# YuemingJin/STswinCL

Hardware: AMD Instinct MI355X
Metric: input frames/s, TswinPlus fwd+bwd+Adam, 4-frame 512x512 clips (higher is better)
Workload: dtype bf16; 1 GPU; BASELINE.json configs[1]: TswinPlus(12) seg train step, 4 clips/GPU x T=4 frames x 3x512x512, swin res (64,64), OHEM-CE, Adam; T=4 because the reference asserts it (swin_512.py:313); clips_per_gpu=4, frames_per_clip=4, parallelism=dp1, graph_requested=True

## Files before the change

### stswincl_amd/csrc/headops.hip

```cpp
#include "common.h"
#include <cstdlib>

static int reduce_rows_per_chunk(int group_rows, int other_blocks, int nrl) {
  int rpc = 8 * nrl;
  while (rpc < 64 * nrl && (long)other_blocks * ((group_rows + 2 * rpc - 1) / (2 * rpc)) >= 1024) rpc *= 2;
  return rpc;
}
static int bn_bwd_rows(long rows_all_groups, int col_blocks, int nrl, int max_rows) {
  static const int tgt_red = getenv("STSWIN_BN_RED_WGS") ? atoi(getenv("STSWIN_BN_RED_WGS")) : 512;
  static const int tgt_dx = getenv("STSWIN_BN_DX_WGS") ? atoi(getenv("STSWIN_BN_DX_WGS")) : 2048;
  const int tgt = max_rows > 32 ? tgt_red : tgt_dx;
  int rows = 8;
  while (rows < max_rows && (long)col_blocks * (rows_all_groups / ((long)2 * rows * nrl)) >= tgt) rows *= 2;
  return rows;
}

DEVI long group_row0(int g, int ch, int rows_per_chunk, int group_rows, int unit, int G) {
  if (unit <= 0) return (long)g * group_rows;
  return ((long)((ch * rows_per_chunk) / unit) * (G - 1) + g) * unit;
}
DEVI long group_first_row(int g, int group_rows, int unit) { return unit > 0 ? (long)g * unit : (long)g * group_rows; }
static int fit_chunk(int rpc, int unit) {
  if (unit <= 0) return rpc;
  while (rpc > 1 && unit % rpc) rpc >>= 1;
// ... 301 lines not shown
  w1 = s - (float)i0;
}

template <typename T>
__global__ __launch_bounds__(256) void bilinear_fwd_kernel(const T* in, long ldi, T* out, long ldo, int F, int h, int w,
                                                            int H, int W, int C) {
  constexpr int PACK = TT<T>::PACK;
  const int ppr = C / PACK;
  const long idx = (long)blockIdx.x * 256 + threadIdx.x;
  if (idx >= (long)F * H * W * ppr) return;
  const int c = (idx % ppr) * PACK;
  const long px = idx / ppr;
  const int x = px % W, y = (px / W) % H, f = px / ((long)W * H);
  int y0, y1, x0, x1; float wy, wx;
  bil_src(y, (float)h / H, h, y0, y1, wy);
  bil_src(x, (float)w / W, w, x0, x1, wx);
  const T* b = in + ((long)f * h * w) * ldi + c;
  Vec16<T> p00, p01, p10, p11, o;
  p00.v = *(const decltype(o.v)*)(b + ((long)y0 * w + x0) * ldi);
  p01.v = *(const decltype(o.v)*)(b + ((long)y0 * w + x1) * ldi);
  p10.v = *(const decltype(o.v)*)(b + ((long)y1 * w + x0) * ldi);
  p11.v = *(const decltype(o.v)*)(b + ((long)y1 * w + x1) * ldi);
#pragma unroll
  for (int e = 0; e < PACK; ++e)
    o.set(e, (1.f - wy) * ((1.f - wx) * p00.get(e) + wx * p01.get(e)) + wy * ((1.f - wx) * p10.get(e) + wx * p11.get(e)));
  *(decltype(o.v)*)(out + px * ldo + c) = o.v;
}

template <typename T>
__global__ __launch_bounds__(256) void bilinear_bwd_kernel(const T* dout, long ldo, T* din, long ldi, int F, int h, int w,
                                                            int H, int W, int C) {
  constexpr int PACK = TT<T>::PACK;
  const int ppr = C / PACK;
  const long idx = (long)blockIdx.x * 256 + threadIdx.x;
  if (idx >= (long)F * h * w * ppr) return;
  const int c = (idx % ppr) * PACK;
  const long px = idx / ppr;
  const int xi = px % w, yi = (px / w) % h, f = px / ((long)w * h);
  const float sy = (float)h / H, sx = (float)w / W;
  const int ylo = max(0, (int)floorf(((float)yi - 0.5f) / sy - 0.5f) - 1), yhi = min(H - 1, (int)ceilf(((float)yi + 1.5f) / sy - 0.5f) + 1);
  const int xlo = max(0, (int)floorf(((float)xi - 0.5f) / sx - 0.5f) - 1), xhi = min(W - 1, (int)ceilf(((float)xi + 1.5f) / sx - 0.5f) + 1);
  float acc[8] = {0, 0, 0, 0, 0, 0, 0, 0};
  for (int y = ylo; y <= yhi; ++y) {
    int y0, y1; float wy;
    bil_src(y, sy, h, y0, y1, wy);
    const float cy = (y0 == yi ? 1.f - wy : 0.f) + (y1 == yi ? wy : 0.f);
    if (cy == 0.f) continue;
    for (int x = xlo; x <= xhi; ++x) {
      int x0, x1; float wx;
      bil_src(x, sx, w, x0, x1, wx);
      const float cx = (x0 == xi ? 1.f - wx : 0.f) + (x1 == xi ? wx : 0.f);
      if (cx == 0.f) continue;
      Vec16<T> d;
      d.v = *(const decltype(d.v)*)(dout + (((long)f * H + y) * W + x) * ldo + c);
#pragma unroll
      for (int e = 0; e < PACK; ++e) acc[e] += cy * cx * d.get(e);
    }
  }
  Vec16<T> o;
#pragma unroll
  for (int e = 0; e < PACK; ++e) o.set(e, acc[e]);
  *(decltype(o.v)*)(din + px * ldi + c) = o.v;
}

template <typename T, typename TO>
__global__ __launch_bounds__(256) void logits_up_fwd_kernel(const T* in, long ldi, TO* out, int F, int h, int w, int H, int W,
                                                             int nc) {
  const long px = (long)blockIdx.x * 256 + threadIdx.x;
  if (px >= (long)F * H * W) return;
  const int x = px % W, y = (px / W) % H, f = px / ((long)W * H);
  int y0, y1, x0, x1; float wy, wx;
  bil_src(y, (float)h / H, h, y0, y1, wy);
  bil_src(x, (float)w / W, w, x0, x1, wx);
  const T* b = in + ((long)f * h * w) * ldi;
  const T* p00 = b + ((long)y0 * w + x0) * ldi; const T* p01 = b + ((long)y0 * w + x1) * ldi;
  const T* p10 = b + ((long)y1 * w + x0) * ldi; const T* p11 = b + ((long)y1 * w + x1) * ldi;
  for (int c = 0; c < nc; ++c) {
    const float v = (1.f - wy) * ((1.f - wx) * to_f32<T>(p00[c]) + wx * to_f32<T>(p01[c])) +
                    wy * ((1.f - wx) * to_f32<T>(p10[c]) + wx * to_f32<T>(p11[c]));
    out[(((long)f * nc + c) * H + y) * W + x] = from_f32<TO>(v);
  }
}

template <typename T, typename TO>
__global__ __launch_bounds__(256) void logits_up_bwd_kernel(const TO* dout, T* din, long ldi, int F, int h, int w, int H, int W,
                                                             int nc) {
  const long idx = (long)blockIdx.x * 256 + threadIdx.x;
  const long npx = (long)F * h * w;
  if (idx >= npx * nc) return;
  const int c = (int)(idx / npx);
  const long px = idx - (long)c * npx;
  const int xi = px % w, yi = (px / w) % h, f = px / ((long)w * h);
  const float sy = (float)h / H, sx = (float)w / W;
  const int ylo = max(0, (int)floorf(((float)yi - 0.5f) / sy - 0.5f) - 1), yhi = min(H - 1, (int)ceilf(((float)yi + 1.5f) / sy - 0.5f) + 1);
  const int xlo = max(0, (int)floorf(((float)xi - 0.5f) / sx - 0.5f) - 1), xhi = min(W - 1, (int)ceilf(((float)xi + 1.5f) / sx - 0.5f) + 1);
  const TO* plane = dout + ((long)f * nc + c) * H * W;
  float acc = 0.f;
  for (int y = ylo; y <= yhi; ++y) {
    int y0, y1; float wy;
    bil_src(y, sy, h, y0, y1, wy);
    const float cy = (y0 == yi ? 1.f - wy : 0.f) + (y1 == yi ? wy : 0.f);
    if (cy == 0.f) continue;
    float row = 0.f;
    for (int x = xlo; x <= xhi; ++x) {
      int x0, x1; float wx;
      bil_src(x, sx, w, x0, x1, wx);
      const float cx = (x0 == xi ? 1.f - wx : 0.f) + (x1 == xi ? wx : 0.f);
      if (cx != 0.f) row += cx * to_f32<TO>(plane[(long)y * W + x]);
    }
    acc += cy * row;
  }
  din[px * ldi + c] = from_f32<T>(acc);
}

DEVI unsigned long long loss_to_fix(float v) { return (unsigned long long)((double)fmaxf(v, 0.f) * 4294967296.0); }
DEVI float fix_to_loss(unsigned long long f) { return (float)((double)f * (1.0 / 4294967296.0)); }

template <typename TL>
__global__ __launch_bounds__(256) void ce_fwd_kernel(const TL* logits, const long* labels, float* loss, float* stats, int F,
                                                      long HW, int nc, int ignore_index, float thresh) {
  float hc = 0.f, hs = 0.f, nbad = 0.f;
  const long n = (long)F * HW;
  for (long px = (long)blockIdx.x * 256 + threadIdx.x; px < n; px += (long)gridDim.x * 256) {
    float l = 0.f;
    const long f = px / HW, p = px % HW;
    const long lab = labels[px];
    if (lab != ignore_index && (lab < 0 || lab >= nc)) {
      l = __builtin_nanf("");
      nbad += 1.f;
    } else if (lab != ignore_index) {
      const TL* b = logits + f * nc * HW + p;
      float mx = -3.0e38f;
      int am = 0;
      for (int c = 0; c < nc; ++c) {
        const float v = to_f32<TL>(b[(long)c * HW]);
        if (v > mx) { mx = v; am = c; }
      }
      float s = 0.f;
      for (int c = 0; c < nc; ++c)
        if (c != am) s += expf(to_f32<TL>(b[(long)c * HW]) - mx);
      l = (mx - to_f32<TL>(b[lab * HW])) + log1pf(s);
    }
    loss[px] = l;
    if (l > thresh) { hc += 1.f; hs += l; }
  }
  float cnt = wave_sum(hc), sm = wave_sum(hs), bad = wave_sum(nbad);
  __shared__ float red[3][4];
  if ((threadIdx.x & 63) == 0) { red[0][threadIdx.x >> 6] = cnt; red[1][threadIdx.x >> 6] = sm; red[2][threadIdx.x >> 6] = bad; }
  __syncthreads();
  if (threadIdx.x == 0) {
    const float nb = red[2][0] + red[2][1] + red[2][2] + red[2][3];
    if (nb != 0.f) atomicAdd(stats + 1, nb);
    atomicAdd(stats + 0, red[0][0] + red[0][1] + red[0][2] + red[0][3]);
    atomicAdd((unsigned long long*)(stats + 2), loss_to_fix(red[1][0] + red[1][1] + red[1][2] + red[1][3]));
  }
}

template <typename TL>
__global__ __launch_bounds__(256) void ce_bwd_kernel(const TL* logits, const long* labels, const float* loss, const float* sel,
                                                      const float* gscale, TL* dlogits, int F, long HW, int nc,
                                                      int ignore_index) {
  const long px = (long)blockIdx.x * 256 + threadIdx.x;
  if (px >= (long)F * HW) return;
  const long f = px / HW, p = px % HW;
  const long lab = labels[px];
  const float l = loss[px];
  const float w = l > sel[0] ? sel[1] : (l == sel[0] ? sel[3] : 0.f);
  const float wgt = (w != 0.f && lab != ignore_index && lab >= 0 && lab < nc) ? w * gscale[0] : 0.f;
  const TL* b = logits + f * nc * HW + p;
  TL* d = dlogits + f * nc * HW + p;
  if (wgt == 0.f) {
    for (int c = 0; c < nc; ++c) d[(long)c * HW] = from_f32<TL>(0.f);
    return;
  }
  float mx = -3.0e38f;
  for (int c = 0; c < nc; ++c) mx = fmaxf(mx, to_f32<TL>(b[(long)c * HW]));
  float s = 0.f;
  for (int c = 0; c < nc; ++c) s += expf(to_f32<TL>(b[(long)c * HW]) - mx);
  const float inv = 1.f / s;
  for (int c = 0; c < nc; ++c) {
    const float pr = expf(to_f32<TL>(b[(long)c * HW]) - mx) * inv;
    d[(long)c * HW] = from_f32<TL>(wgt * (pr - (c == lab ? 1.f : 0.f)));
  }
}

#define PACK_OF(dt) ((dt) == 0 ? 8 : 4)
#define DISPATCH_T(dt, CALL_BF16, CALL_F32) do { if ((dt) == 0) { CALL_BF16; } else { CALL_F32; } } while (0)

static int colstats_geometry(int dtype, int M, int C, int groups, int unit_rows, int* cpb_o, int* rpc_o, int* cpg_o) {
  if (C % PACK_OF(dtype) || groups <= 0 || M % groups) return -1401;
  if (unit_rows > 0 && M % ((long)groups * unit_rows)) return -1405;
  const int ppr = C / PACK_OF(dtype), cpb = pick_cpb(ppr);
  const int gr = M / groups, rpc = fit_chunk(reduce_rows_per_chunk(gr, groups * ((ppr + cpb - 1) / cpb), 256 / cpb), unit_rows);
  if (rpc <= 0) return -1405;
  *cpb_o = cpb; *rpc_o = rpc; *cpg_o = (gr + rpc - 1) / rpc;
  return 0;
}
extern "C" long stswin_colstats_scratch(int dtype, int M, int C, int groups, int unit_rows) {
  int cpb, rpc, cpg;
  const int rc = colstats_geometry(dtype, M, C, groups, unit_rows, &cpb, &rpc, &cpg);
  return rc ? rc : (long)groups * cpg * 2 * C;
}

extern "C" int stswin_colstats(int dtype, const void* x, long ldx, float* sum, float* sumsq, int M, int C, int groups,
                               int unit_rows, float* scratch, void* stream) {
  int cpb, rpc, cpg;
  const int rc = colstats_geometry(dtype, M, C, groups, unit_rows, &cpb, &rpc, &cpg);
  if (rc) return rc;
  if (ldx % PACK_OF(dtype)) return -1401;
  if (!scratch) return -1406;
  const int ppr = C / PACK_OF(dtype), gr = M / groups;
  dim3 grid((ppr + cpb - 1) / cpb, groups * cpg);
  hipStream_t st = (hipStream_t)stream;
  if (sumsq)
    DISPATCH_T(dtype, hipLaunchKernelGGL((colstats_kernel<bf16, true>), grid, dim3(256), 0, st, (const bf16*)x, ldx, scratch, C, gr, cpg, rpc, cpb, unit_rows),
               hipLaunchKernelGGL((colstats_kernel<float, true>), grid, dim3(256), 0, st, (const float*)x, ldx, scratch, C, gr, cpg, rpc, cpb, unit_rows));
  else
    DISPATCH_T(dtype, hipLaunchKernelGGL((colstats_kernel<bf16, false>), grid, dim3(256), 0, st, (const bf16*)x, ldx, scratch, C, gr, cpg, rpc, cpb, unit_rows),
               hipLaunchKernelGGL((colstats_kernel<float, false>), grid, dim3(256), 0, st, (const float*)x, ldx, scratch, C, gr, cpg, rpc, cpb, unit_rows));
  const int rf = stswin_fold_launch(scratch, 2L * C, (long)cpg * 2 * C, cpg, C, sumsq ? 2 : 1, sum, sumsq, nullptr, C, groups, 1, st);
  if (rf) return rf;
  STSWIN_CHECK_LAUNCH();
  return 0;
}

extern "C" int stswin_bn_finalize(int dtype, const void* x, long ldx, const float* sum, const float* sumsq, float* mean,
                                  float* rstd, float* running_mean, float* running_var, int M, int C, int groups, float eps,
                                  float momentum, int unit_rows, void* stream) {
  if (groups <= 0 || M % groups) return -1401;
  hipStream_t st = (hipStream_t)stream;
  dim3 grid((C + 255) / 256);
  DISPATCH_T(dtype, hipLaunchKernelGGL(bn_finalize_kernel<bf16>, grid, dim3(256), 0, st, (const bf16*)x, ldx, sum, sumsq, mean, rstd, running_mean, running_var, C, groups, M / groups, eps, momentum, unit_rows),
             hipLaunchKernelGGL(bn_finalize_kernel<float>, grid, dim3(256), 0, st, (const float*)x, ldx, sum, sumsq, mean, rstd, running_mean, running_var, C, groups, M / groups, eps, momentum, unit_rows));
  STSWIN_CHECK_LAUNCH();
  return 0;
}

extern "C" int stswin_bn_apply(int dtype, const void* x, long ldx, const float* mean, const float* rstd, const float* gamma,
                               const float* beta, const void* resid, long ldr, void* y, long ldy, int M, int C, int groups,
                               int relu, int unit_rows, void* stream) {
  const int pk = PACK_OF(dtype);
  if (C % pk || ldx % pk || ldy % pk || (resid && ldr % pk) || groups <= 0 || M % groups) return -1402;
  const int ppr = C / pk, cpb = pick_cpb(ppr);
  if (unit_rows > 0 && M % ((long)groups * unit_rows)) return -1405;
  const int gr = M / groups, rpc = fit_chunk(8 * (256 / cpb), unit_rows);
  if (rpc <= 0) return -1405;
  const int cpg = (gr + rpc - 1) / rpc;
  dim3 grid((ppr + cpb - 1) / cpb, groups * cpg);
  hipStream_t st = (hipStream_t)stream;
  DISPATCH_T(dtype, hipLaunchKernelGGL(bn_apply_kernel<bf16>, grid, dim3(256), 0, st, (const bf16*)x, ldx, mean, rstd, gamma, beta, (const bf16*)resid, ldr, (bf16*)y, ldy, C, gr, cpg, rpc, relu, cpb, unit_rows),
             hipLaunchKernelGGL(bn_apply_kernel<float>, grid, dim3(256), 0, st, (const float*)x, ldx, mean, rstd, gamma, beta, (const float*)resid, ldr, (float*)y, ldy, C, gr, cpg, rpc, relu, cpb, unit_rows));
  STSWIN_CHECK_LAUNCH();
  return 0;
}

static int bn_bwd_geometry(int dtype, int M, int C, int groups, int unit_rows, int* cpb_o, int* rpc_o, int* rpc2_o) {
  const int pk = PACK_OF(dtype);
  if (C % pk || groups <= 0 || M % groups) return -1403;
  if (unit_rows > 0 && M % ((long)groups * unit_rows)) return -1405;
  const int ppr = C / pk, cpb = pick_cpb(ppr), xb = (ppr + cpb - 1) / cpb, nrl = 256 / cpb;
  const int rpc = fit_chunk(bn_bwd_rows(M, xb, nrl, 64) * nrl, unit_rows);
  const int rpc2 = fit_chunk(bn_bwd_rows(M, xb, nrl, 32) * nrl, unit_rows);
  if (rpc <= 0 || rpc2 <= 0) return -1405;
  *cpb_o = cpb; *rpc_o = rpc; *rpc2_o = rpc2;
  return 0;
}
extern "C" long stswin_bn_bwd_scratch(int dtype, int M, int C, int groups, int unit_rows) {
  int cpb, rpc, rpc2;
  const int rc = bn_bwd_geometry(dtype, M, C, groups, unit_rows, &cpb, &rpc, &rpc2);
// ... 77 lines not shown
          const int kx = ix - 2 * ox;
          if (kx < 0 || kx > 2) continue;
          const int o = oy * 2 + ox;
          const unsigned char t = (unsigned char)(ky * 3 + kx);
#pragma unroll
          for (int e = 0; e < PACK; ++e) {
            const float u = z.get(e);
            if (u > best[o][e] || ba[o][e] == 255) { best[o][e] = u; ba[o][e] = t; }
          }
        }
      }
    }
  }
#pragma unroll
  for (int oy = 0; oy < 2; ++oy)
#pragma unroll
    for (int ox = 0; ox < 2; ++ox) {
      const int yo = 2 * yb + oy, xo = 2 * xb + ox, o = oy * 2 + ox;
      if (yo >= Hp || xo >= Wp) continue;
      const long px = (f * Hp + yo) * Wp + xo;
      Vec16<T> r;
      unsigned a[2] = {0, 0};
#pragma unroll
      for (int e = 0; e < PACK; ++e) { r.set(e, best[o][e]); a[e >> 2] |= (unsigned)ba[o][e] << (8 * (e & 3)); }
      if (PACK == 8) *(uint2*)(arg + px * C + c) = uint2{a[0], a[1]};
      else *(unsigned*)(arg + px * C + c) = a[0];
      *(decltype(r.v)*)(out + px * ldo + c) = r.v;
    }
}

extern "C" int stswin_bn_relu_pool(int dtype, const void* x, long ldx, const float* mean, const float* rstd, const float* gamma,
                                   const float* beta, void* out, long ldo, unsigned char* arg, int frames, int H, int W, int C, int groups,
                                   int unit_rows, void* stream) {
  const int pk = PACK_OF(dtype);
  const long M = (long)frames * H * W;
  if (frames <= 0 || H <= 0 || W <= 0 || C % pk || ldx % pk || ldo % pk || groups <= 0 || M % groups) return -1408;
  if (unit_rows > 0 ? (unit_rows % ((long)H * W) != 0 || M % ((long)groups * unit_rows)) : ((M / groups) % ((long)H * W) != 0)) return -1408;
  const int Hp = (H - 1) / 2 + 1, Wp = (W - 1) / 2 + 1;
  const long n = (long)frames * ((Hp + 1) / 2) * ((Wp + 1) / 2) * (C / pk);
  dim3 grid((unsigned)((n + 255) / 256));
  hipStream_t st = (hipStream_t)stream;
  DISPATCH_T(dtype, hipLaunchKernelGGL(bn_relu_pool_kernel<bf16>, grid, dim3(256), 0, st, (const bf16*)x, ldx, mean, rstd, gamma, beta, (bf16*)out, ldo, arg, frames, H, W, Hp, Wp, C, groups, (int)(M / groups), unit_rows),
             hipLaunchKernelGGL(bn_relu_pool_kernel<float>, grid, dim3(256), 0, st, (const float*)x, ldx, mean, rstd, gamma, beta, (float*)out, ldo, arg, frames, H, W, Hp, Wp, C, groups, (int)(M / groups), unit_rows));
  STSWIN_CHECK_LAUNCH();
  return 0;
}

extern "C" int stswin_rows_broadcast(int dtype, const float* v, void* out, long ldo, int M, int C, int groups, float scale,
                                     int accumulate, void* stream) {
  const int pk = PACK_OF(dtype);
  if (C % pk || ldo % pk || groups <= 0 || M % groups) return -1404;
  const long n = (long)M * (C / pk);
  dim3 grid((unsigned)((n + 255) / 256));
  hipStream_t st = (hipStream_t)stream;
  DISPATCH_T(dtype, hipLaunchKernelGGL(rows_broadcast_kernel<bf16>, grid, dim3(256), 0, st, v, (bf16*)out, ldo, M, C, M / groups, scale, accumulate),
             hipLaunchKernelGGL(rows_broadcast_kernel<float>, grid, dim3(256), 0, st, v, (float*)out, ldo, M, C, M / groups, scale, accumulate));
  STSWIN_CHECK_LAUNCH();
  return 0;
}

extern "C" int stswin_bilinear(int dtype, const void* in, long ldi, void* out, long ldo, int frames, int h, int w, int H, int W,
                               int C, int backward, void* stream) {
  const int pk = PACK_OF(dtype);
  if (C % pk || ldi % pk || ldo % pk) return -1405;
  hipStream_t st = (hipStream_t)stream;
  if (!backward) {
    const long n = (long)frames * H * W * (C / pk);
    dim3 grid((unsigned)((n + 255) / 256));
    DISPATCH_T(dtype, hipLaunchKernelGGL(bilinear_fwd_kernel<bf16>, grid, dim3(256), 0, st, (const bf16*)in, ldi, (bf16*)out, ldo, frames, h, w, H, W, C),
               hipLaunchKernelGGL(bilinear_fwd_kernel<float>, grid, dim3(256), 0, st, (const float*)in, ldi, (float*)out, ldo, frames, h, w, H, W, C));
  } else {
    const long n = (long)frames * h * w * (C / pk);
    dim3 grid((unsigned)((n + 255) / 256));
    DISPATCH_T(dtype, hipLaunchKernelGGL(bilinear_bwd_kernel<bf16>, grid, dim3(256), 0, st, (const bf16*)in, ldi, (bf16*)out, ldo, frames, h, w, H, W, C),
               hipLaunchKernelGGL(bilinear_bwd_kernel<float>, grid, dim3(256), 0, st, (const float*)in, ldi, (float*)out, ldo, frames, h, w, H, W, C));
  }
  STSWIN_CHECK_LAUNCH();
  return 0;
}

extern "C" int stswin_logits_upsample(int dtype, const void* tokens, long ldt, void* nchw, int frames, int h, int w, int H,
                                      int W, int nc, int backward, void* stream) {
  hipStream_t st = (hipStream_t)stream;
  if (!backward) {
    const long n = (long)frames * H * W;
    dim3 grid((unsigned)((n + 255) / 256));
    DISPATCH_T(dtype, hipLaunchKernelGGL((logits_up_fwd_kernel<bf16, bf16>), grid, dim3(256), 0, st, (const bf16*)tokens, ldt, (bf16*)nchw, frames, h, w, H, W, nc),
               hipLaunchKernelGGL((logits_up_fwd_kernel<float, float>), grid, dim3(256), 0, st, (const float*)tokens, ldt, (float*)nchw, frames, h, w, H, W, nc));
  } else {
    const long n = (long)frames * h * w * nc;
    dim3 grid((unsigned)((n + 255) / 256));
    DISPATCH_T(dtype, hipLaunchKernelGGL((logits_up_bwd_kernel<bf16, bf16>), grid, dim3(256), 0, st, (const bf16*)nchw, (bf16*)tokens, ldt, frames, h, w, H, W, nc),
               hipLaunchKernelGGL((logits_up_bwd_kernel<float, float>), grid, dim3(256), 0, st, (const float*)nchw, (float*)tokens, ldt, frames, h, w, H, W, nc));
  }
  STSWIN_CHECK_LAUNCH();
  return 0;
}

extern "C" int stswin_ce_fwd(int dtype, const void* logits, const long* labels, float* loss, float* stats, int frames, long HW,
                             int nc, int ignore_index, float thresh, void* stream) {
  const long n = (long)frames * HW;
  const long want = (n + 255) / 256;
  dim3 grid((unsigned)(want < 1024 ? want : 1024));
  hipStream_t st = (hipStream_t)stream;
  DISPATCH_T(dtype, hipLaunchKernelGGL(ce_fwd_kernel<bf16>, grid, dim3(256), 0, st, (const bf16*)logits, labels, loss, stats, frames, HW, nc, ignore_index, thresh),
             hipLaunchKernelGGL(ce_fwd_kernel<float>, grid, dim3(256), 0, st, (const float*)logits, labels, loss, stats, frames, HW, nc, ignore_index, thresh));
  STSWIN_CHECK_LAUNCH();
  return 0;
}

extern "C" int stswin_ce_bwd(int dtype, const void* logits, const long* labels, const float* loss, const float* sel,
                             const float* gscale, void* dlogits, int frames, long HW, int nc, int ignore_index, void* stream) {
  const long n = (long)frames * HW;
  dim3 grid((unsigned)((n + 255) / 256));
  hipStream_t st = (hipStream_t)stream;
  DISPATCH_T(dtype, hipLaunchKernelGGL(ce_bwd_kernel<bf16>, grid, dim3(256), 0, st, (const bf16*)logits, labels, loss, sel, gscale, (bf16*)dlogits, frames, HW, nc, ignore_index),
             hipLaunchKernelGGL(ce_bwd_kernel<float>, grid, dim3(256), 0, st, (const float*)logits, labels, loss, sel, gscale, (float*)dlogits, frames, HW, nc, ignore_index));
  STSWIN_CHECK_LAUNCH();
  return 0;
}

struct OhemWork {
  unsigned cnt[3][2048];
  unsigned long long sum[3][2048];
  unsigned long long sabove[3];
  unsigned state[3][2];
};

__device__ void ohem_scan(const unsigned* cnt, const unsigned long long* sum, int nbins, unsigned k, unsigned* out ,
                          unsigned long long* out_sum ) {
  __shared__ unsigned pc[256];
  __shared__ unsigned long long ps[256];
  const int t = threadIdx.x, per = nbins / 256;
  unsigned c = 0;
  unsigned long long sm = 0;
  for (int b = 0; b < per; ++b) { c += cnt[nbins - 1 - (t * per + b)]; sm += sum[nbins - 1 - (t * per + b)]; }
  pc[t] = c; ps[t] = sm;
  __syncthreads();
  for (int d = 1; d < 256; d <<= 1) {
    const unsigned c2 = t >= d ? pc[t - d] : 0u;
    const unsigned long long s2 = t >= d ? ps[t - d] : 0ull;
    __syncthreads();
    pc[t] += c2; ps[t] += s2;
    __syncthreads();
  }
  const unsigned incl = pc[t], excl = incl - c;
  if (excl < k && k <= incl) {
    unsigned above = excl;
    unsigned long long sabove = ps[t] - sm;
    for (int b = 0; b < per; ++b) {
      const int bin = nbins - 1 - (t * per + b);
      const unsigned cb = cnt[bin];
      if (above + cb >= k) { out[0] = (unsigned)bin; out[1] = k - above; out_sum[0] = sabove; break; }
      above += cb; sabove += sum[bin];
    }
  }
  __syncthreads();
}

__global__ __launch_bounds__(256) void ohem_hist_kernel(const float* loss, long n, long n_min, const float* stats, OhemWork* wk, int level) {
  if (stats[0] > (float)n_min) return;
  __shared__ unsigned hc[2048];
  __shared__ unsigned long long hs[2048];
  __shared__ unsigned sc[2];
  __shared__ unsigned long long ssum[1];
  for (int i = threadIdx.x; i < 2048; i += 256) { hc[i] = 0u; hs[i] = 0ull; }
  unsigned prefix = 0;
  if (level > 0) {
    const unsigned k = level == 1 ? (unsigned)n_min : wk->state[1][1];
    ohem_scan(wk->cnt[level - 1], wk->sum[level - 1], 2048, k, sc, ssum);
    const unsigned up = level == 1 ? 0u : wk->state[1][0];
    prefix = level == 1 ? sc[0] : ((up << 11) | sc[0]);
    if (blockIdx.x == 0 && threadIdx.x == 0) {
      const unsigned long long sprev = level == 1 ? 0ull : wk->sabove[1];
      wk->state[level][0] = prefix; wk->state[level][1] = sc[1]; wk->sabove[level] = sprev + ssum[0];
    }
  }
  __syncthreads();
  const int shift = level == 0 ? 21 : (level == 1 ? 10 : 0);
  const unsigned mask = level == 2 ? 1023u : 2047u;
  for (long i = (long)blockIdx.x * 256 + threadIdx.x; i < n; i += (long)gridDim.x * 256) {
    const float v = loss[i];
    const unsigned key = __float_as_uint(v) & 0x7fffffffu;
    const bool in = level == 0 || (level == 1 ? (key >> 21) == prefix : (key >> 10) == prefix);
    if (in) { const unsigned b = (key >> shift) & mask; atomicAdd(&hc[b], 1u); atomicAdd(&hs[b], loss_to_fix(v)); }
  }
  __syncthreads();
  for (int i = threadIdx.x; i < 2048; i += 256)
    if (hc[i]) { atomicAdd(&wk->cnt[level][i], hc[i]); atomicAdd(&wk->sum[level][i], hs[i]); }
}

__global__ __launch_bounds__(256) void ohem_final_kernel(long n_min, float thresh, const float* stats, const OhemWork* wk, float* value,
                                                         float* sel) {
  const float n_hard = stats[0];
  const bool bad = stats[1] != 0.f;
  if (n_hard > (float)n_min) {
    if (threadIdx.x == 0) {
      const float inv = 1.f / fmaxf(n_hard, 1.f);
// ... 3421 lines not shown
```

### stswincl_amd/csrc/rowops.hip

```cpp
#include "common.h"
#include <cstdlib>

DEVI int win_src_token(int r, int T, int H, int W, int ws, int shift, int f0, int frames_total) {
  const int N = ws * ws, nwx = W / ws, nW = (H / ws) * nwx;
  const int n = r % N; int q = r / N;
  const int t = q % T; q /= T;
  const int wi = q % nW; const int b = q / nW;
  const int ys = (wi / nwx) * ws + n / ws, xs = (wi % nwx) * ws + n % ws;
  int y = ys + shift, x = xs + shift;
  if (y >= H) y -= H;
  if (x >= W) x -= W;
  return ((b * frames_total + f0 + t) * H + y) * W + x;
}

__global__ void win_rowmap_kernel(int* map, int rows, int T, int H, int W, int ws, int shift, int f0, int ftot) {
  const int r = blockIdx.x * blockDim.x + threadIdx.x;
  if (r < rows) map[r] = win_src_token(r, T, H, W, ws, shift, f0, ftot);
}

template <typename T>
__global__ __launch_bounds__(256) void win_move_kernel(const T* in, T* out, int rows, int C, int Tt, int H, int W,
                                                        int ws, int shift, int f0, int ftot, int dir) {
  constexpr int PACK = TT<T>::PACK;
  const int r = blockIdx.x * 4 + (threadIdx.x >> 6);
// ... 495 lines not shown
      const int c = (p * 64 + l) * PACK;
      if (c < C) {
        Vec16<T> xi, di;
        xi.v = __builtin_bit_cast(vec_t, cur.xi[p]); di.v = __builtin_bit_cast(vec_t, cur.di[p]);
        float gm[PACK];
#pragma unroll
        for (int e = 0; e < PACK; e += 4) *(f32x4*)(gm + e) = *(const f32x4*)(sgam + c + e);
#pragma unroll
        for (int e = 0; e < PACK; ++e) {
          const float d = di.get(e);
          const float xh = (xi.get(e) - mu) * rs;
          const float g = d * gm[e];
          s1 += g;
          s2 += g * xh;
          dg[p][e] += d * xh;
          db[p][e] += d;
        }
      }
    }
    s1 = wave_sum(s1) / C;
    s2 = wave_sum(s2) / C;
#pragma unroll
    for (int p = 0; p < NP; ++p) {
      const int c = (p * 64 + l) * PACK;
      if (c < C) {
        const int s = c / Cseg, cc = c - s * Cseg;
        const long row = rows ? (long)rows[(long)s * M + r] : (long)r;
        T* dst = dx + row * lddx + cc;
        Vec16<T> xi, di, o;
        xi.v = __builtin_bit_cast(vec_t, cur.xi[p]); di.v = __builtin_bit_cast(vec_t, cur.di[p]);
        if constexpr (EARLY) o.v = __builtin_bit_cast(vec_t, cur.old[p]);
        else if constexpr (ACC) o.v = *(const vec_t*)(add + row * ldadd + cc);
        float gm[PACK];
#pragma unroll
        for (int e = 0; e < PACK; e += 4) *(f32x4*)(gm + e) = *(const f32x4*)(sgam + c + e);
#pragma unroll
        for (int e = 0; e < PACK; ++e) {
          const float xh = (xi.get(e) - mu) * rs;
          const float g = di.get(e) * gm[e];
          const float val = rs * (g - s1 - xh * s2);
          const float fin = ACC ? o.get(e) + val : val;
          o.set(e, fin);
          if constexpr (DXS) ds[p][e] += fin;
        }
        *(vec_t*)dst = o.v;
      }
    }
  }
  }
  float* sg = (float*)smem;
  float* rep = ws + (long)blockIdx.x * 3 * C;
  auto fold = [&](const float (&acc)[NP][PACK], float* out) __attribute__((always_inline)) {
#pragma unroll
    for (int p = 0; p < NP; ++p) {
      const int c = (p * 64 + l) * PACK;
      if (c < C) {
#pragma unroll
        for (int e = 0; e < PACK; ++e) sg[w * C + c + e] = acc[p][e];
      }
    }
    __syncthreads();
    for (int c = threadIdx.x; c < C; c += NW * 64) {
      float t = sg[c];
#pragma unroll
      for (int k = 1; k < NW; ++k) t += sg[k * C + c];
      out[c] = t;
    }
    __syncthreads();
  };
  fold(dg, rep);
  fold(db, rep + C);
  if constexpr (DXS) fold(ds, rep + 2 * C);
}

template <typename T>
__global__ __launch_bounds__(256) void colsum_kernel(const T* y, long ldy, float* part, int M, int N, int rows_per_block) {
  constexpr int PACK = TT<T>::PACK;
  __shared__ float red[8][32 * 8];
  const int cp = threadIdx.x & 31, rl = threadIdx.x >> 5;
  const int c = (blockIdx.x * 32 + cp) * PACK;
  float acc[8] = {0, 0, 0, 0, 0, 0, 0, 0};
  const int r0 = blockIdx.y * rows_per_block;
  if (c < N) {
    for (int r = r0 + rl; r < min(M, r0 + rows_per_block); r += 8) {
      Vec16<T> in;
      in.v = *(const decltype(in.v)*)(y + (long)r * ldy + c);
#pragma unroll
      for (int e = 0; e < PACK; ++e) acc[e] += in.get(e);
    }
  }
#pragma unroll
  for (int e = 0; e < 8; ++e) red[rl][cp * 8 + e] = acc[e];
  __syncthreads();
  if (rl == 0 && c < N) {
#pragma unroll
    for (int e = 0; e < PACK; ++e) {
      float t = 0.f;
#pragma unroll
      for (int k = 0; k < 8; ++k) t += red[k][cp * 8 + e];
      part[(long)blockIdx.y * N + c + e] = t;
    }
  }
}

__global__ __launch_bounds__(256) void vec_gather_kernel(const float* v, const int* map, float* out, int n, float fill) {
  const int i = blockIdx.x * 256 + threadIdx.x;
  if (i < n) { const int j = map[i]; out[i] = j >= 0 ? v[j] : fill; }
}

struct VecGatherMulti { const float* v[4]; float* out[4]; float fill[4]; const int* map; int n; };
__global__ __launch_bounds__(256) void vec_gather_multi_kernel(VecGatherMulti p) {
  const int i = blockIdx.x * 256 + threadIdx.x, k = blockIdx.y;
  if (i < p.n) { const int j = p.map[i]; p.out[k][i] = j >= 0 ? p.v[k][j] : p.fill[k]; }
}

__global__ __launch_bounds__(256) void bias_expand_kernel(const float* table, const long* index, const float* mask, float* out,
                                                          int N, int heads, int nW) {
  const long n = (long)nW * heads * N * N;
  for (long t = (long)blockIdx.x * 256 + threadIdx.x; t < n; t += (long)gridDim.x * 256) {
    const int i = (int)(t % N), j = (int)((t / N) % N);
    const int h = (int)((t / ((long)N * N)) % heads), w = (int)(t / ((long)N * N * heads));
    float v = table[index[(long)i * N + j] * heads + h];
    if (mask) v += mask[((long)w * N + i) * N + j];
    out[t] = v;
  }
}
#define BEM_MAX 16
struct BiasExpandMulti { const float* table[BEM_MAX]; const long* index[BEM_MAX]; const float* mask[BEM_MAX]; float* out[BEM_MAX];
                         int N[BEM_MAX], heads[BEM_MAX], nW[BEM_MAX]; };
__global__ __launch_bounds__(256) void bias_expand_multi_kernel(BiasExpandMulti p) {
  const int e = blockIdx.y, N = p.N[e], heads = p.heads[e];
  const float* table = p.table[e]; const long* index = p.index[e]; const float* mask = p.mask[e]; float* out = p.out[e];
  const long n = (long)p.nW[e] * heads * N * N;
  for (long t = (long)blockIdx.x * 256 + threadIdx.x; t < n; t += (long)gridDim.x * 256) {
    const int i = (int)(t % N), j = (int)((t / N) % N);
    const int h = (int)((t / ((long)N * N)) % heads), w = (int)(t / ((long)N * N * heads));
    float v = table[index[(long)i * N + j] * heads + h];
    if (mask) v += mask[((long)w * N + i) * N + j];
    out[t] = v;
  }
}
__global__ __launch_bounds__(256) void bias_scatter_kernel(const float* dbiasT, const int* order, const int* offs, float* dtable, int N,
                                                            int heads, int table_rows, int nslabs) {
  const int t = blockIdx.x * 4 + (threadIdx.x >> 6), l = threadIdx.x & 63;
  if (t >= table_rows * heads) return;
  const int e = t / heads, h = t - e * heads;
  const long NN = (long)N * N;
  float acc = 0.f;
  for (int q = offs[e] + l; q < offs[e + 1]; q += 64) {
    const int pr = order[q], i = pr / N, j = pr - i * N;
    const float* src = dbiasT + ((long)h * N + j) * N + i;
    for (int sl = 0; sl < nslabs; ++sl) acc += src[(long)sl * heads * NN];
  }
#pragma unroll
  for (int d = 32; d >= 1; d >>= 1) acc += __shfl_xor(acc, d);
  if (l == 0) dtable[(long)e * heads + h] += acc;
}

extern "C" int stswin_win_rowmap(int* map, int B, int T, int H, int W, int ws, int shift, int f0, int frames_total,
                                 void* stream) {
  if (H % ws || W % ws || shift < 0 || shift >= ws) return -1101;
  const int rows = B * T * H * W;
  hipLaunchKernelGGL(win_rowmap_kernel, dim3((rows + 255) / 256), dim3(256), 0, (hipStream_t)stream, map, rows, T, H, W,
                     ws, shift, f0, frames_total);
  STSWIN_CHECK_LAUNCH();
  return 0;
}

extern "C" int stswin_win_move(int dtype, const void* in, void* out, int B, int T, int H, int W, int C, int ws, int shift,
                               int f0, int frames_total, int dir, void* stream) {
  if (H % ws || W % ws || shift < 0 || shift >= ws) return -1101;
// ... 809 lines not shown
```

Measured before the change: 611.4 frames/s.

## Tile logits-upsample backward in LDS, vectorize OHEM CE kernels, unroll colsum loads

Adds an LDS-tiled backward for the bilinear logits upsample. Each block stages the needed source rows once and reuses precomputed separable weights, replacing per-output strided gathers. Adds vectorized cross-entropy forward and backward kernels that process four pixels per thread with 16-byte loads, and a single-pass log-softmax. The column-sum kernel now issues 16 row loads before accumulating, for more memory-level parallelism. These target head and loss bandwidth and latency costs, but add complexity, LDS use and fallback paths.

```diff
diff --git a/stswincl_amd/csrc/headops.hip b/stswincl_amd/csrc/headops.hip
--- a/stswincl_amd/csrc/headops.hip
+++ b/stswincl_amd/csrc/headops.hip
@@ -407,6 +407,19 @@
   }
 }
 
+#define HEAD_NC_MAX 16
+template <typename T> struct Vec4;
+template <> struct Vec4<bf16> {
+  bf16x4 v;
+  DEVI float get(int i) const { return (float)v[i]; }
+  DEVI void set(int i, float f) { v[i] = (bf16)f; }
+};
+template <> struct Vec4<float> {
+  f32x4 v;
+  DEVI float get(int i) const { return v[i]; }
+  DEVI void set(int i, float f) { v[i] = f; }
+};
+
 template <typename T, typename TO>
 __global__ __launch_bounds__(256) void logits_up_bwd_kernel(const TO* dout, T* din, long ldi, int F, int h, int w, int H, int W,
                                                              int nc) {
@@ -438,6 +451,110 @@
   din[px * ldi + c] = from_f32<T>(acc);
 }
 
+DEVI int up_bwd_lo(int i, float s) { return max(0, (int)floorf(((float)i - 0.5f) / s - 0.5f) - 1); }
+DEVI int up_bwd_hi(int i, float s, int N) { return min(N - 1, (int)ceilf(((float)i + 1.5f) / s - 0.5f) + 1); }
+DEVI float up_bwd_weight(int dst, float s, int n_in, int i) {
+  int i0, i1; float w1;
+  bil_src(dst, s, n_in, i0, i1, w1);
+  return (i0 == i ? 1.f - w1 : 0.f) + (i1 == i ? w1 : 0.f);
+}
+#define UP_BWD_TY 8
+#define UP_BWD_TX 32
+#define UP_BWD_CLS 1
+#define UP_BWD_NPT 12
+template <typename T, typename TO>
+__global__ __launch_bounds__(256) void logits_up_bwd_tile_kernel(const TO* dout, T* din, long ldi, int F, int h, int w, int H, int W,
+                                                                  int nc, int lds_rows, int lds_pitch, int wx_max, int wy_max) {
+  constexpr int P = TT<TO>::PACK, TY = UP_BWD_TY, TX = UP_BWD_TX, NR = 8, NPT = UP_BWD_NPT;
+  extern __shared__ __attribute__((aligned(16))) char up_bwd_lds[];
+  TO* tile = (TO*)up_bwd_lds;
+  float* rowsum = (float*)(up_bwd_lds + (size_t)lds_rows * lds_pitch * sizeof(TO));
+  float* wxt = rowsum + lds_rows * TX;
+  float* wyt = wxt + wx_max * TX;
+  const int tiles_x = (w + TX - 1) / TX;
+  const int xi0 = (blockIdx.x % tiles_x) * TX, yi0 = (blockIdx.x / tiles_x) * TY;
+  const int c0 = blockIdx.y * UP_BWD_CLS, ncls = min(UP_BWD_CLS, nc - c0), f = blockIdx.z;
+  const int tx = threadIdx.x % TX, ty = threadIdx.x / TX;
+  const int xi = xi0 + tx, yi = yi0 + ty;
+  const bool live = xi < w && yi < h;
+  const float sy = (float)h / H, sx = (float)w / W;
+  const int ybase = up_bwd_lo(yi0, sy), yend = up_bwd_hi(min(yi0 + TY, h) - 1, sy, H);
+  const int xa = up_bwd_lo(xi0, sx) / P * P, xe = min(W, (up_bwd_hi(min(xi0 + TX, w) - 1, sx, W) / P + 1) * P);
+  const int nrows = yend - ybase + 1, ppr = (xe - xa) / P, npieces = nrows * ppr;
+  const int xlo = up_bwd_lo(min(xi, w - 1), sx), nwx = up_bwd_hi(min(xi, w - 1), sx, W) - xlo + 1;
+  const int ylo = up_bwd_lo(min(yi, h - 1), sy), nwy = up_bwd_hi(min(yi, h - 1), sy, H) - ylo + 1;
+  const bool fits = nrows <= lds_rows && ppr * P <= lds_pitch && npieces <= NPT * 256 && nwx <= wx_max && nwy <= wy_max;
+  if (__syncthreads_or(!fits)) {
+    if (live)
+      for (int c = c0; c < c0 + ncls; ++c) {
+        const TO* plane = dout + ((long)f * nc + c) * H * W;
+        float acc = 0.f;
+        for (int j = 0; j < nwy; ++j) {
+          const float cy = up_bwd_weight(ylo + j, sy, h, yi);
+          if (cy == 0.f) continue;
+          float row = 0.f;
+          for (int i = 0; i < nwx; ++i) {
+            const float cx = up_bwd_weight(xlo + i, sx, w, xi);
+            if (cx != 0.f) row += cx * to_f32<TO>(plane[(long)(ylo + j) * W + xlo + i]);
+          }
+          acc += cy * row;
+        }
+        din[(((long)f * h + yi) * w + xi) * ldi + c] = from_f32<T>(acc);
+      }
+    return;
+  }
+  for (int i = ty; i < nwx; i += TY) wxt[i * TX + tx] = xi < w ? up_bwd_weight(xlo + i, sx, w, xi) : 0.f;
+  for (int j = tx; j < nwy; j += TX) wyt[j * TY + ty] = yi < h ? up_bwd_weight(ylo + j, sy, h, yi) : 0.f;
+  Vec16<TO> pre[NPT];
+  auto request = [&](int c) {
+    const TO* plane = dout + ((long)f * nc + c) * H * W;
+#pragma unroll
+    for (int u = 0; u < NPT; ++u) {
+      const int i = threadIdx.x + u * 256;
+      if (i < npieces) pre[u].v = *(const decltype(pre[u].v)*)(plane + (long)(ybase + i / ppr) * W + xa + (i % ppr) * P);
+    }
+  };
+  request(c0);
+  for (int cc = 0; cc < ncls; ++cc) {
+#pragma unroll
+    for (int u = 0; u < NPT; ++u) {
+      const int i = threadIdx.x + u * 256;
+      if (i < npieces) *(decltype(pre[u].v)*)(tile + (i / ppr) * lds_pitch + (i % ppr) * P) = pre[u].v;
+    }
+    __syncthreads();
+    if (cc + 1 < ncls) request(c0 + cc + 1);
+    if (xi < w) {
+      const TO* col = tile + (xlo - xa);
+      for (int rb = ty; rb < nrows; rb += TY * NR) {
+        float row[NR];
+#pragma unroll
+        for (int r = 0; r < NR; ++r) row[r] = 0.f;
+        for (int i = 0; i < nwx; ++i) {
+          const float cx = wxt[i * TX + tx];
+          if (cx != 0.f) {
+#pragma unroll
+            for (int r = 0; r < NR; ++r)
+              if (rb + r * TY < nrows) row[r] += cx * to_f32<TO>(col[(rb + r * TY) * lds_pitch + i]);
+          }
+        }
+#pragma unroll
+        for (int r = 0; r < NR; ++r)
+          if (rb + r * TY < nrows) rowsum[(rb + r * TY) * TX + tx] = row[r];
+      }
+    }
+    __syncthreads();
+    if (live) {
+      float acc = 0.f;
+      for (int j = 0; j < nwy; ++j) {
+        const float cy = wyt[j * TY + ty];
+        if (cy == 0.f) continue;
+        acc += cy * rowsum[(ylo - ybase + j) * TX + tx];
+      }
+      din[(((long)f * h + yi) * w + xi) * ldi + c0 + cc] = from_f32<T>(acc);
+    }
+  }
+}
+
 DEVI unsigned long long loss_to_fix(float v) { return (unsigned long long)((double)fmaxf(v, 0.f) * 4294967296.0); }
 DEVI float fix_to_loss(unsigned long long f) { return (float)((double)f * (1.0 / 4294967296.0)); }
 
@@ -509,7 +626,152 @@
   }
 }
 
+#define CE_NC_MAX HEAD_NC_MAX
+#define CE_PX 4
+typedef long i64x2 __attribute__((ext_vector_type(2)));
+
+template <typename TL>
+DEVI float ce_pixel_loss(const Vec4<TL>* v, int e, long lab, int nc, int ignore_index, float& nbad) {
+  if (lab != ignore_index && (lab < 0 || lab >= nc)) { nbad += 1.f; return __builtin_nanf(""); }
+  if (lab == ignore_index) return 0.f;
+  float mx = -3.0e38f, xl = 0.f;
+  int am = 0;
+#pragma unroll
+  for (int c = 0; c < CE_NC_MAX; ++c)
+    if (c < nc) {
+      const float x = v[c].get(e);
+      if (x > mx) { mx = x; am = c; }
+      if (c == lab) xl = x;
+    }
+  float s = 0.f;
+#pragma unroll
+  for (int c = 0; c < CE_NC_MAX; ++c)
+    if (c < nc && c != am) s += expf(v[c].get(e) - mx);
+  return (mx - xl) + log1pf(s);
+}
+
+template <typename TL>
+__global__ __launch_bounds__(1024) void ce_fwd_quad_kernel(const TL* logits, const long* labels, float* loss, float* stats, long n,
+                                                            long HW, int nc, int ignore_index, float thresh, int vgrid) {
+  constexpr int P = CE_PX;
+  __shared__ __attribute__((aligned(16))) float lc[4][4][256];
+  __shared__ float red[4][3][4];
+  __shared__ unsigned long long vfix[4];
+  __shared__ float vcnt[4], vbad[4];
+  const int vq = threadIdx.x >> 8, t = threadIdx.x & 255, kk = t >> 6, j = t & 63;
+  const long stride = (long)vgrid * 256;
+  const int vb0 = blockIdx.x * 4, vb = vb0 + vq;
+  const long first = (long)vb * 256;
+  const int nk = vb < vgrid ? (int)((n - first + stride - 1) / stride) : 0;
+  const int nk0 = (int)((n - (long)vb0 * 256 + stride - 1) / stride);
+  float hc = 0.f, nbad = 0.f, hs = 0.f;
+  for (int k0 = 0; k0 < nk0; k0 += 4) {
+    const long px = first + (long)(k0 + kk) * stride + j * P;
+    float l[P];
+    if (k0 + kk < nk && px < n) {
+      const long f = px / HW, p = px % HW;
+      const TL* b = logits + f * nc * HW + p;
+      const i64x2 la = *(const i64x2*)(labels + px), lb = *(const i64x2*)(labels + px + 2);
+      const long lab[P] = {la[0], la[1], lb[0], lb[1]};
+      Vec4<TL> v[CE_NC_MAX];
+#pragma unroll
+      for (int c = 0; c < CE_NC_MAX; ++c)
+        if (c < nc) v[c].v = *(const decltype(v[c].v)*)(b + (long)c * HW);
+#pragma unroll
+      for (int e = 0; e < P; ++e) {
+        l[e] = ce_pixel_loss<TL>(v, e, lab[e], nc, ignore_index, nbad);
+        if (l[e] > thresh) hc += 1.f;
+      }
+      *(f32x4*)(loss + px) = f32x4{l[0], l[1], l[2], l[3]};
+    } else {
+#pragma unroll
+      for (int e = 0; e < P; ++e) l[e] = __builtin_nanf("");
+    }
+    *(f32x4*)&lc[vq][kk][j * P] = f32x4{l[0], l[1], l[2], l[3]};
+    __syncthreads();
+#pragma unroll
+    for (int q = 0; q < 4; ++q) {
+      const float a = lc[vq][q][t];
+      if (a > thresh) hs += a;
+    }
+    __syncthreads();
+  }
+  const float cnt = wave_sum(hc), bad = wave_sum(nbad), sm = wave_sum(hs);
+  if (j == 0) { red[vq][0][kk] = cnt; red[vq][1][kk] = sm; red[vq][2][kk] = bad; }
+  __syncthreads();
+  if (t == 0) {
+    vbad[vq] = red[vq][2][0] + red[vq][2][1] + red[vq][2][2] + red[vq][2][3];
+    vcnt[vq] = red[vq][0][0] + red[vq][0][1] + red[vq][0][2] + red[vq][0][3];
+    vfix[vq] = loss_to_fix(red[vq][1][0] + red[vq][1][1] + red[vq][1][2] + red[vq][1][3]);
+  }
+  __syncthreads();
+  if (threadIdx.x == 0) {
+    const float nb = vbad[0] + vbad[1] + vbad[2] + vbad[3];
+    if (nb != 0.f) atomicAdd(stats + 1, nb);
+    atomicAdd(stats + 0, vcnt[0] + vcnt[1] + vcnt[2] + vcnt[3]);
+    atomicAdd((unsigned long long*)(stats + 2), vfix[0] + vfix[1] + vfix[2] + vfix[3]);
+  }
+}
+
+template <typename TL>
+__global__ __launch_bounds__(256) void ce_bwd_quad_kernel(const TL* logits, const long* labels, const float* loss, const float* sel,
+                                                           const float* gscale, TL* dlogits, long n, long HW, int nc,
+                                                           int ignore_index) {
+  constexpr int P = CE_PX;
+  const long px = ((long)blockIdx.x * 256 + threadIdx.x) * P;
+  if (px >= n) return;
+  const long f = px / HW, p = px % HW;
+  const float s0 = sel[0], s1 = sel[1], s3 = sel[3], gs = gscale[0];
+  const i64x2 la = *(const i64x2*)(labels + px), lb = *(const i64x2*)(labels + px + 2);
+  const long lab[P] = {la[0], la[1], lb[0], lb[1]};
+  const f32x4 l4 = *(const f32x4*)(loss + px);
+  float wgt[P];
+  bool any = false;
+#pragma unroll
+  for (int e = 0; e < P; ++e) {
+    const float l = l4[e];
+    const float w = l > s0 ? s1 : (l == s0 ? s3 : 0.f);
+    wgt[e] = (w != 0.f && lab[e] != ignore_index && lab[e] >= 0 && lab[e] < nc) ? w * gs : 0.f;
+    any = any || wgt[e] != 0.f;
+  }
+  const TL* b = logits + f * nc * HW + p;
+  TL* d = dlogits + f * nc * HW + p;
+  Vec4<TL> v[CE_NC_MAX];
+  if (any) {
+#pragma unroll
+    for (int c = 0; c < CE_NC_MAX; ++c)
+      if (c < nc) v[c].v = *(const decltype(v[c].v)*)(b + (long)c * HW);
+  }
+#pragma unroll
+  for (int e = 0; e < P; ++e) {
+    if (wgt[e] == 0.f) {
+#pragma unroll
+      for (int c = 0; c < CE_NC_MAX; ++c) v[c].set(e, 0.f);
+      continue;
+    }
+    float mx = -3.0e38f;
+#pragma unroll
+    for (int c = 0; c < CE_NC_MAX; ++c)
+      if (c < nc) mx = fmaxf(mx, v[c].get(e));
+    float ex[CE_NC_MAX];
+    float s = 0.f;
+#pragma unroll
+    for (int c = 0; c < CE_NC_MAX; ++c)
+      if (c < nc) { ex[c] = expf(v[c].get(e) - mx); s += ex[c]; }
+    const float inv = 1.f / s;
+#pragma unroll
+    for (int c = 0; c < CE_NC_MAX; ++c)
+      if (c < nc) v[c].set(e, wgt[e] * (ex[c] * inv - (c == lab[e] ? 1.f : 0.f)));
+  }
+#pragma unroll
+  for (int c = 0; c < CE_NC_MAX; ++c)
+    if (c < nc) *(decltype(v[c].v)*)(d + (long)c * HW) = v[c].v;
+}
+
 #define PACK_OF(dt) ((dt) == 0 ? 8 : 4)
+static inline bool aligned16(const void* p) { return ((uintptr_t)p & 15) == 0; }
+static int up_bwd_lo_host(int i, float s) { const int v = (int)floorf(((float)i - 0.5f) / s - 0.5f) - 1; return v > 0 ? v : 0; }
+static int up_bwd_hi_host(int i, float s, int N) { const int v = (int)ceilf(((float)i + 1.5f) / s - 0.5f) + 1; return v < N - 1 ? v : N - 1; }
 #define DISPATCH_T(dt, CALL_BF16, CALL_F32) do { if ((dt) == 0) { CALL_BF16; } else { CALL_F32; } } while (0)
 
 static int colstats_geometry(int dtype, int M, int C, int groups, int unit_rows, int* cpb_o, int* rpc_o, int* cpg_o) {
@@ -753,16 +1015,42 @@
 extern "C" int stswin_logits_upsample(int dtype, const void* tokens, long ldt, void* nchw, int frames, int h, int w, int H,
                                       int W, int nc, int backward, void* stream) {
   hipStream_t st = (hipStream_t)stream;
+  const int pk = PACK_OF(dtype);
+  const bool pieces = frames > 0 && h > 0 && w > 0 && H > 0 && nc > 0 && W > 0 && W % pk == 0 && aligned16(nchw);
   if (!backward) {
     const long n = (long)frames * H * W;
     dim3 grid((unsigned)((n + 255) / 256));
     DISPATCH_T(dtype, hipLaunchKernelGGL((logits_up_fwd_kernel<bf16, bf16>), grid, dim3(256), 0, st, (const bf16*)tokens, ldt, (bf16*)nchw, frames, h, w, H, W, nc),
                hipLaunchKernelGGL((logits_up_fwd_kernel<float, float>), grid, dim3(256), 0, st, (const float*)tokens, ldt, (float*)nchw, frames, h, w, H, W, nc));
   } else {
-    const long n = (long)frames * h * w * nc;
-    dim3 grid((unsigned)((n + 255) / 256));
-    DISPATCH_T(dtype, hipLaunchKernelGGL((logits_up_bwd_kernel<bf16, bf16>), grid, dim3(256), 0, st, (const bf16*)nchw, (bf16*)tokens, ldt, frames, h, w, H, W, nc),
-               hipLaunchKernelGGL((logits_up_bwd_kernel<float, float>), grid, dim3(256), 0, st, (const float*)nchw, (float*)tokens, ldt, frames, h, w, H, W, nc));
+    int rows = 0, pitch = 0, wxm = 0, wym = 0;
+    size_t lds = 0;
+    if (pieces && nc <= 65535 * UP_BWD_CLS && frames <= 65535) {
+      const float sy = (float)h / H, sx = (float)w / W;
+      for (int y0 = 0; y0 < h; y0 += UP_BWD_TY) {
+        const int r = up_bwd_hi_host((y0 + UP_BWD_TY < h ? y0 + UP_BWD_TY : h) - 1, sy, H) - up_bwd_lo_host(y0, sy) + 1;
+        if (r > rows) rows = r;
+      }
+      for (int x0 = 0; x0 < w; x0 += UP_BWD_TX) {
+        const int xa = up_bwd_lo_host(x0, sx) / pk * pk;
+        int xe = (up_bwd_hi_host((x0 + UP_BWD_TX < w ? x0 + UP_BWD_TX : w) - 1, sx, W) / pk + 1) * pk;
+        if (xe > W) xe = W;
+        if (xe - xa > pitch) pitch = xe - xa;
+      }
+      for (int i = 0; i < h; ++i) { const int n = up_bwd_hi_host(i, sy, H) - up_bwd_lo_host(i, sy) + 1; if (n > wym) wym = n; }
+      for (int i = 0; i < w; ++i) { const int n = up_bwd_hi_host(i, sx, W) - up_bwd_lo_host(i, sx) + 1; if (n > wxm) wxm = n; }
+      lds = (size_t)rows * pitch * (dtype == 0 ? 2 : 4) + ((size_t)rows * UP_BWD_TX + (size_t)wxm * UP_BWD_TX + (size_t)wym * UP_BWD_TY) * sizeof(float);
+    }
+    if (rows > 0 && pitch > 0 && lds <= 64 * 1024 && (long)rows * (pitch / pk) <= UP_BWD_NPT * 256) {
+      dim3 grid((unsigned)(((w + UP_BWD_TX - 1) / UP_BWD_TX) * ((h + UP_BWD_TY - 1) / UP_BWD_TY)), (unsigned)((nc + UP_BWD_CLS - 1) / UP_BWD_CLS), (unsigned)frames);
+      DISPATCH_T(dtype, hipLaunchKernelGGL((logits_up_bwd_tile_kernel<bf16, bf16>), grid, dim3(256), lds, st, (const bf16*)nchw, (bf16*)tokens, ldt, frames, h, w, H, W, nc, rows, pitch, wxm, wym),
+                 hipLaunchKernelGGL((logits_up_bwd_tile_kernel<float, float>), grid, dim3(256), lds, st, (const float*)nchw, (float*)tokens, ldt, frames, h, w, H, W, nc, rows, pitch, wxm, wym));
+    } else {
+      const long n = (long)frames * h * w * nc;
+      dim3 grid((unsigned)((n + 255) / 256));
+      DISPATCH_T(dtype, hipLaunchKernelGGL((logits_up_bwd_kernel<bf16, bf16>), grid, dim3(256), 0, st, (const bf16*)nchw, (bf16*)tokens, ldt, frames, h, w, H, W, nc),
+                 hipLaunchKernelGGL((logits_up_bwd_kernel<float, float>), grid, dim3(256), 0, st, (const float*)nchw, (float*)tokens, ldt, frames, h, w, H, W, nc));
+    }
   }
   STSWIN_CHECK_LAUNCH();
   return 0;
@@ -774,6 +1062,12 @@
   const long want = (n + 255) / 256;
   dim3 grid((unsigned)(want < 1024 ? want : 1024));
   hipStream_t st = (hipStream_t)stream;
+  if (n > 0 && nc <= CE_NC_MAX && HW % CE_PX == 0 && aligned16(logits) && aligned16(labels) && aligned16(loss)) {
+    const int vgrid = (int)grid.x;
+    dim3 gq((unsigned)((vgrid + 3) / 4));
+    DISPATCH_T(dtype, hipLaunchKernelGGL(ce_fwd_quad_kernel<bf16>, gq, dim3(1024), 0, st, (const bf16*)logits, labels, loss, stats, n, HW, nc, ignore_index, thresh, vgrid),
+               hipLaunchKernelGGL(ce_fwd_quad_kernel<float>, gq, dim3(1024), 0, st, (const float*)logits, labels, loss, stats, n, HW, nc, ignore_index, thresh, vgrid));
+  } else
   DISPATCH_T(dtype, hipLaunchKernelGGL(ce_fwd_kernel<bf16>, grid, dim3(256), 0, st, (const bf16*)logits, labels, loss, stats, frames, HW, nc, ignore_index, thresh),
              hipLaunchKernelGGL(ce_fwd_kernel<float>, grid, dim3(256), 0, st, (const float*)logits, labels, loss, stats, frames, HW, nc, ignore_index, thresh));
   STSWIN_CHECK_LAUNCH();
@@ -785,6 +1079,11 @@
   const long n = (long)frames * HW;
   dim3 grid((unsigned)((n + 255) / 256));
   hipStream_t st = (hipStream_t)stream;
+  if (n > 0 && nc <= CE_NC_MAX && HW % CE_PX == 0 && aligned16(logits) && aligned16(labels) && aligned16(loss) && aligned16(dlogits)) {
+    dim3 gv((unsigned)((n / CE_PX + 255) / 256));
+    DISPATCH_T(dtype, hipLaunchKernelGGL(ce_bwd_quad_kernel<bf16>, gv, dim3(256), 0, st, (const bf16*)logits, labels, loss, sel, gscale, (bf16*)dlogits, n, HW, nc, ignore_index),
+               hipLaunchKernelGGL(ce_bwd_quad_kernel<float>, gv, dim3(256), 0, st, (const float*)logits, labels, loss, sel, gscale, (float*)dlogits, n, HW, nc, ignore_index));
+  } else
   DISPATCH_T(dtype, hipLaunchKernelGGL(ce_bwd_kernel<bf16>, grid, dim3(256), 0, st, (const bf16*)logits, labels, loss, sel, gscale, (bf16*)dlogits, frames, HW, nc, ignore_index),
              hipLaunchKernelGGL(ce_bwd_kernel<float>, grid, dim3(256), 0, st, (const float*)logits, labels, loss, sel, gscale, (float*)dlogits, frames, HW, nc, ignore_index));
   STSWIN_CHECK_LAUNCH();
diff --git a/stswincl_amd/csrc/rowops.hip b/stswincl_amd/csrc/rowops.hip
--- a/stswincl_amd/csrc/rowops.hip
+++ b/stswincl_amd/csrc/rowops.hip
@@ -601,11 +601,19 @@
   float acc[8] = {0, 0, 0, 0, 0, 0, 0, 0};
   const int r0 = blockIdx.y * rows_per_block;
   if (c < N) {
-    for (int r = r0 + rl; r < min(M, r0 + rows_per_block); r += 8) {
-      Vec16<T> in;
-      in.v = *(const decltype(in.v)*)(y + (long)r * ldy + c);
-#pragma unroll
-      for (int e = 0; e < PACK; ++e) acc[e] += in.get(e);
+    constexpr int U = 16;
+    const int r_end = min(M, r0 + rows_per_block);
+    for (int r = r0 + rl; r < r_end; r += 8 * U) {
+      Vec16<T> in[U];
+#pragma unroll
+      for (int u = 0; u < U; ++u)
+        if (r + 8 * u < r_end) in[u].v = *(const decltype(in[u].v)*)(y + (long)(r + 8 * u) * ldy + c);
+#pragma unroll
+      for (int u = 0; u < U; ++u)
+        if (r + 8 * u < r_end) {
+#pragma unroll
+          for (int e = 0; e < PACK; ++e) acc[e] += in[u].get(e);
+        }
     }
   }
 #pragma unroll
```

Measured after the change: 615.6 frames/s, median of 6. Within noise of the previous version (+0.7%).
